# jgrss/cultionet

Measured on AMD Instinct MI355X. Metric: train_chips_per_sec, higher is better.
Workload: dtype f32

## Files before the change

### cultionet_amd/csrc/cn_conv.hip

```cpp
#include "cn_common.h"
#include "cn_conv_geom.h"
#include "cn_profile.h"

#include <cstdlib>

#define KC 8

static int cn_reduce_slices(const CnConvGeom& g, hipStream_t stream);

template <int TN, int TM>
__device__ __forceinline__ void cn_igemm_epilogue(const CnConvGeom& g, const f32x16 (&acc)[TN][TM],
                                                  const bool (&pix_ok)[TM], const int (&out_off)[TM], int co_base,
                                                  int half, int grp, int split, int b,
                                                  const float* __restrict__ bias, float* __restrict__ y) {
  const int HWout = g.Hout * g.Wout;
  const bool sliced = g.slice_stride != 0;
  float* yb = sliced ? g.part + (long)(grp * g.splits + split) * g.slice_stride + (long)b * g.Cout * HWout
                     : y + (long)b * g.ybs;
  const bool first = split == 0;
#pragma unroll
  for (int tn = 0; tn < TN; ++tn) {
#pragma unroll
    for (int r = 0; r < 16; ++r) {
      const int co = co_base + tn * 32 + (r & 3) + 8 * (r >> 2) + 4 * half;
// ... 166 lines not shown
  {                                                                                                        \
    const float* wrow = w_lds + ((t_) * KC + half) * NT + wn * (TN * 32) + l31;                            \
    _Pragma("unroll") for (int tn = 0; tn < TN; ++tn) opa[bf_][tn] = wrow[(2 * (cp_)) * NT + tn * 32];     \
    opb[bf_][0] = in_lds[pix_lds[0] + (2 * (cp_)) * plane + (toff_)];                                      \
    opb[bf_][1] = in_lds[pix_lds[1] + (2 * (cp_)) * plane + (toff_)];                                      \
  }
#define CN_MFMA(bf_)                                                                                       \
  _Pragma("unroll") for (int tn = 0; tn < TN; ++tn) _Pragma("unroll") for (int tm = 0; tm < 2; ++tm)       \
      acc[tn][tm] = __builtin_amdgcn_mfma_f32_32x32x2f32(opa[bf_][tn], opb[bf_][tm], acc[tn][tm], 0, 0, 0);
      int toff_cur = tap_lds[0];
      CN_LOAD_OPS(0, 0, 0, toff_cur);
#pragma unroll 1
      for (int t = 0; t < ntaps; ++t) {
        const int toff_nxt = (t + 1 < ntaps) ? tap_lds[t + 1] : 0;
        CN_LOAD_OPS(1, t, 1, toff_cur);
        CN_MFMA(0);
        CN_LOAD_OPS(0, t, 2, toff_cur);
        CN_MFMA(1);
        CN_LOAD_OPS(1, t, 3, toff_cur);
        CN_MFMA(0);
        if (t + 1 < ntaps) CN_LOAD_OPS(0, t + 1, 0, toff_nxt);
        CN_MFMA(1);
        toff_cur = toff_nxt;
      }
#undef CN_LOAD_OPS
#undef CN_MFMA
    }
#undef CN_PREFETCH
  }

  cn_igemm_epilogue<TN, 2>(g, acc, pix_ok, out_off, n0 + wn * (TN * 32), half, grp, split, b, bias, y);
}

template <int WAVES_N, int TN, int TM, int NV, int RP>
__global__ __launch_bounds__(256, (NV <= 1 ? 2 : 1)) void cn_conv_igemm_vec_kernel(const CnConvGeom g) {
  constexpr int WAVES_M = 4 / WAVES_N;
  constexpr int MT = WAVES_M * TM * 32;
  constexpr int NT = WAVES_N * TN * 32;
  constexpr int WI = (CN_MAX_TAPS * KC * (NT / 4) + 255) / 256;
  constexpr int VS = NV * 1024;
  constexpr bool PADR = RP == 1 || RP == 2;
  constexpr int ODD = RP == 3 ? 1 : 0;
  constexpr int VSS = VS + ODD;
  extern __shared__ __attribute__((aligned(16))) float smem[];
  float* in_lds = smem;
  float* w_lds = smem + g.w_lds_off;
  int* tap_lds = reinterpret_cast<int*>(smem + g.tap_lds_off);

  const int tid = threadIdx.x, lane = tid & 63, wid = tid >> 6;
  const int half = lane >> 5, l31 = lane & 31;
  const int wm = wid / WAVES_N, wn = wid % WAVES_N;

  int bx, by, split;
  if (!cn_xcd_block(g.grid_x, g.grid_y, g.grid_x * g.grid_y * g.splits, bx, by, split)) return;
  int ci_ = 0;
  if (g.interleave) {
    ci_ = bx % g.ncls;
  } else {
#pragma unroll 1
    for (int c = 1; c < g.ncls; ++c)
      if (bx >= g.cls[c].block_begin) ci_ = c;
  }
  const int grp = g.cls[ci_].grp;
  const float* __restrict__ x = g.gx[grp];
  const float* __restrict__ wp = g.gwp[grp];
  const float* __restrict__ bias = g.gbias[grp];
  float* __restrict__ y = g.gy[grp];
  const int Hg = g.cls[ci_].Hg, Wg = g.cls[ci_].Wg, ntaps = g.cls[ci_].ntaps;
  const int vplane = g.cls[ci_].vplane;
  const int min_dy = g.cls[ci_].min_dy, min_dx = g.cls[ci_].min_dx;
  const int oy0 = g.cls[ci_].oy0, ox0 = g.cls[ci_].ox0;
  const int tiles_per_img = g.cls[ci_].tiles_per_img;
  const int tile = g.interleave ? bx / g.ncls : bx - g.cls[ci_].block_begin;
  const int b = tile / tiles_per_img;
  const int m0 = (tile - b * tiles_per_img) * MT;
  const int Win = g.Win;
  const int pitch = PADR ? ((Win + 3) / 4 * 4 + 4) : Win;
  if (tid < ntaps) {
    tap_lds[tid] = PADR ? (g.cls[ci_].dy[tid] - min_dy) * pitch + g.cls[ci_].dx[tid]
                      : (g.cls[ci_].dy[tid] - min_dy) * Win + (g.cls[ci_].dx[tid] - min_dx);
    tap_lds[CN_MAX_TAPS + tid] = g.cls[ci_].wt[tid];
    tap_lds[2 * CN_MAX_TAPS + tid] = g.cls[ci_].dx[tid];
  }
  __syncthreads();
  const int n0 = by * NT;
  const int Mimg = Hg * Wg;
  const int gy0 = m0 / Wg;
  const int HWin = g.Hin * Win;
  const int start = PADR ? (gy0 * g.is + min_dy) * Win : (gy0 * g.is + min_dy) * Win + min_dx;
  const int f0 = (start >> 2) << 2;
  const int sh = start - f0;

  int goff[NV];
  int ldst[NV];
  int ldst2[NV];
#pragma unroll
  for (int i = 0; i < NV; ++i) {
    const int e4 = 4 * (tid + i * 256) - (PADR ? sh : 0);
    const int lim = PADR ? g.cls[ci_].rows * Win : vplane;
    ldst[i] = 0;
    ldst2[i] = 0;
    if (e4 + 3 >= 0 && e4 < lim) {
      const int fq = start + e4 - (PADR ? 0 : sh);
      goff[i] = (fq >= 0 && (ODD ? fq < HWin : fq + 3 < HWin)) ? fq : -1;
      if (RP == 1) {
        const int r = e4 / Win;
        ldst[i] = r * pitch + 4 + (e4 - r * Win);
      } else if (RP == 2) {
        const int ea = e4 < 0 ? e4 + 2 : e4, eb = e4 + 2;
        const int ra = ea / Win, rb = eb / Win;
        ldst[i] = e4 < 0 ? -1 : ra * pitch + 4 + (ea - ra * Win);
        ldst2[i] = eb < lim ? rb * pitch + 4 + (eb - rb * Win) : -1;
      } else {
        ldst[i] = e4;
      }
    } else {
      goff[i] = -2;
    }
  }
  if (PADR) {
    for (int e = tid; e < KC * VS; e += 256) in_lds[e] = 0.f;
  }

  int pix_lds[TM], out_off[TM];
  unsigned colmask[TM];
  bool pix_ok[TM];
#pragma unroll
  for (int tm = 0; tm < TM; ++tm) {
    const int p = m0 + wm * (TM * 32) + tm * 32 + l31;
    pix_ok[tm] = p < Mimg;
    const int pc = pix_ok[tm] ? p : Mimg - 1;
    const int gy = pc / Wg, gx = pc - gy * Wg;
    pix_lds[tm] = PADR ? ((gy - gy0) * g.is) * pitch + 4 + gx * g.is + half * VS
                     : ((gy - gy0) * g.is) * Win + gx * g.is + sh + half * VSS;
    out_off[tm] = (gy * g.os + oy0) * g.Wout + gx * g.os + ox0;
    unsigned m = 0;
    for (int t = 0; t < ntaps; ++t) {
      const int ix = gx * g.is + tap_lds[2 * CN_MAX_TAPS + t];
      if (ix >= 0 && ix < Win) m |= 1u << t;
    }
    colmask[tm] = m;
  }

  f32x16 acc[TN][TM];
#pragma unroll
  for (int tn = 0; tn < TN; ++tn)
#pragma unroll
    for (int tm = 0; tm < TM; ++tm)
#pragma unroll
      for (int r = 0; r < 16; ++r) acc[tn][tm][r] = 0.f;
  const float* xb = x + (long)b * g.xbs;
  const int nw4 = ntaps * KC * (NT / 4);
  const int nchunks = (g.Cin + KC - 1) / KC;
  int ch = split * g.chunks_per_split;
  int ch_end = ch + g.chunks_per_split;
  if (ch_end > nchunks) ch_end = nchunks;

  if (ntaps > 0 && ch < ch_end) {
    f32x4 xin[KC][NV];
    f32x4 win[WI];
    constexpr unsigned CN_OOB = 0x80000000u;
    const __amdgpu_buffer_rsrc_t xrs =
        __builtin_amdgcn_make_buffer_rsrc(const_cast<float*>(xb), 0, 0x7fffffff, 0x00020000);
    const __amdgpu_buffer_rsrc_t wrs =
        __builtin_amdgcn_make_buffer_rsrc(const_cast<float*>(wp), 0, 0x7fffffff, 0x00020000);
    unsigned xo[NV], wo[WI];
#pragma unroll
    for (int i = 0; i < NV; ++i) xo[i] = goff[i] >= 0 ? (unsigned)goff[i] * 4u : CN_OOB;
#pragma unroll
    for (int j = 0; j < WI; ++j) {
      const int f = tid + j * 256;
      wo[j] = CN_OOB;
      if (f < nw4) {
        const int row = f / (NT / 4), c4 = f - row * (NT / 4);
        const int t = row / KC, ci = row - t * KC;
        wo[j] = (unsigned)(((tap_lds[CN_MAX_TAPS + t] * g.Kpad + ci) * g.Npad + n0 + c4 * 4) * 4);
      }
    }
#define CN_PREFETCH_V(c0_)                                                                                 \
  {                                                                                                        \
    const int c0 = (c0_);                                                                                  \
    _Pragma("unroll") for (int ci = 0; ci < KC; ++ci) {                                                    \
      if ((c0 + ci) < g.Cin) {                                                           \
        const int so = ODD ? (((c0 + ci) * HWin) & ~3) * 4 : (c0 + ci) * HWin * 4;                                                               \
        _Pragma("unroll") for (int i = 0; i < NV; ++i)                                                     \
            xin[ci][i] = __builtin_bit_cast(f32x4, __builtin_amdgcn_raw_buffer_load_b128(xrs, xo[i], so, 0)); \
      } else {                                                                                             \
        _Pragma("unroll") for (int i = 0; i < NV; ++i) xin[ci][i] = f32x4{0.f, 0.f, 0.f, 0.f};             \
      }                                                                                                    \
    }                                                                                                      \
    const int wso = c0 * g.Npad * 4;                                                                       \
    _Pragma("unroll") for (int j = 0; j < WI; ++j)                                                         \
        win[j] = __builtin_bit_cast(f32x4, __builtin_amdgcn_raw_buffer_load_b128(wrs, wo[j], wso, 0));     \
  }
    CN_PREFETCH_V(ch * KC);
    for (; ch < ch_end; ++ch) {
      __syncthreads();
#pragma unroll
      for (int ci = 0; ci < KC; ++ci)
#pragma unroll
        for (int i = 0; i < NV; ++i)
          if (goff[i] != -2) {
            if (RP == 2) {
              if (ldst[i] >= 0) *reinterpret_cast<float2*>(in_lds + ci * VS + ldst[i]) = make_float2(xin[ci][i][0], xin[ci][i][1]);
              if (ldst2[i] >= 0) *reinterpret_cast<float2*>(in_lds + ci * VS + ldst2[i]) = make_float2(xin[ci][i][2], xin[ci][i][3]);
            } else if (ODD) {
              f32x4 v = xin[ci][i];
              const int dl = ci & 3;
              const bool first = dl > 0 && goff[i] == 0;
              const bool last = dl < 3 && goff[i] == HWin - 1;
#pragma unroll
              for (int j = 0; j < 4; ++j)
                if ((first && j < dl) || (last && j > dl)) v[j] = 0.f;
              *reinterpret_cast<f32x4*>(in_lds + ci * VS + (ci & ~3) + ldst[i]) = v;
            } else {
              *reinterpret_cast<f32x4*>(in_lds + ci * VS + ldst[i]) = xin[ci][i];
            }
          }
#pragma unroll
      for (int j = 0; j < WI; ++j) {
        const int f = tid + j * 256;
        if (f < nw4) *reinterpret_cast<f32x4*>(w_lds + f * 4) = win[j];
      }
      __syncthreads();
      if (ch + 1 < ch_end) CN_PREFETCH_V((ch + 1) * KC);
#pragma unroll 1
      for (int t = 0; t < ntaps; ++t) {
        const int toff = tap_lds[t];
        const float* wrow = w_lds + (t * KC + half) * NT + wn * (TN * 32) + l31;
        const float* brow[TM];
        int msk[TM];
#pragma unroll
        for (int tm = 0; tm < TM; ++tm) {
          brow[tm] = in_lds + pix_lds[tm] + toff;
          msk[tm] = PADR ? -1 : __builtin_amdgcn_sbfe((int)colmask[tm], t, 1);
        }
#pragma unroll
        for (int cp = 0; cp < KC / 2; ++cp) {
          float a[TN], bb[TM];
#pragma unroll
          for (int tn = 0; tn < TN; ++tn) a[tn] = wrow[(2 * cp) * NT + tn * 32];
#pragma unroll
          for (int tm = 0; tm < TM; ++tm)
            bb[tm] = PADR ? brow[tm][(2 * cp) * VS] : __int_as_float(__float_as_int(brow[tm][(2 * cp) * VSS]) & msk[tm]);
#pragma unroll
          for (int tn = 0; tn < TN; ++tn)
#pragma unroll
            for (int tm = 0; tm < TM; ++tm)
              acc[tn][tm] = __builtin_amdgcn_mfma_f32_32x32x2f32(a[tn], bb[tm], acc[tn][tm], 0, 0, 0);
        }
      }
    }
#undef CN_PREFETCH_V
  }

  cn_igemm_epilogue<TN, TM>(g, acc, pix_ok, out_off, n0 + wn * (TN * 32), half, grp, split, b, bias, y);
}

__global__ void cn_pack_weights_kernel(const float* __restrict__ w, float* __restrict__ wp, int T, int K,
                                       int N, int Kpad, int Npad, long sk, long sn, long st) {
  const long total = (long)T * Kpad * Npad;
  for (long i = blockIdx.x * (long)blockDim.x + threadIdx.x; i < total; i += (long)gridDim.x * blockDim.x) {
    const int n = (int)(i % Npad);
    const long r = i / Npad;
    const int k = (int)(r % Kpad);
    const int t = (int)(r / Kpad);
    wp[i] = (k < K && n < N) ? w[k * sk + n * sn + t * st] : 0.f;
  }
}

struct CnPackDesc {
  const float* w;
  float* wp;
  int T, K, N, Kpad, Npad;
  long sk, sn, st;
};

#define CN_PK_TS 32
#define CN_PK_PITCH (32 * CN_MAX_TAPS + 1)
__global__ __launch_bounds__(256) void cn_pack_weights_batched_kernel(const CnPackDesc* __restrict__ descs) {
  __shared__ float tile[CN_PK_TS * CN_PK_PITCH];
  const CnPackDesc d = descs[blockIdx.y];
  const bool n_slow = d.sn > d.sk;
  const long ss = n_slow ? d.sn : d.sk, sm = n_slow ? d.sk : d.sn;
  const int S = n_slow ? d.N : d.K, M = n_slow ? d.K : d.N;
  const int Spad = n_slow ? d.Npad : d.Kpad, Mpad = n_slow ? d.Kpad : d.Npad;
  if (d.T > CN_MAX_TAPS || d.st != 1 || sm != d.T) {
    const long total = (long)d.T * d.Kpad * d.Npad;
    for (long i = blockIdx.x * (long)blockDim.x + threadIdx.x; i < total; i += (long)gridDim.x * blockDim.x) {
// ... 139 lines not shown
      if (t == 0 || k.dy[t] > max_dy) max_dy = k.dy[t];
      if (t == 0 || k.dx[t] > max_dx) max_dx = k.dx[t];
    }
    const int rows = (rows_g - 1) * g.is + (max_dy - k.min_dy) + 1;
    k.pitch = (k.Wg - 1) * g.is + (max_dx - k.min_dx) + 1;
    k.plane = rows * k.pitch;
    k.vplane = (rows * g.Win + (max_dx - k.min_dx) + 4 + 3) / 4 * 4;
    k.rows = rows;
    {
      const int rpitch = (g.Win + 3) / 4 * 4 + 4;
      if ((rows + 1) * rpitch + 4 > p.max_rplane) p.max_rplane = (rows + 1) * rpitch + 4;
    }
    if (-k.min_dx > p.max_absdx) p.max_absdx = -k.min_dx;
    if (max_dx > p.max_absdx) p.max_absdx = max_dx;
    k.tiles_per_img = (Mimg + MT - 1) / MT;
    k.block_begin = p.total_tiles;
    p.total_tiles += g.B * k.tiles_per_img;
    if (k.plane > p.max_plane) p.max_plane = k.plane;
    if (k.vplane > p.max_vplane) p.max_vplane = k.vplane;
    if (k.ntaps > p.max_taps) p.max_taps = k.ntaps;
    p.flops += 2.0 * g.B * Mimg * (double)g.Cout * g.Cin * k.ntaps;
  }
  g.interleave = 0;
  if (g.ncls > 1 && g.want_interleave) {
    bool same = true;
    for (int c = 1; c < g.ncls; ++c) same = same && g.cls[c].tiles_per_img == g.cls[0].tiles_per_img;
    g.interleave = same ? 1 : 0;
  }
  return p;
}

struct CnChoice { int cfg, splits, cps; double cost; };

static double cn_launch_cost(long blocks, int cps, double mt_units, int splits, double out_elems) {
  const double F = 273.0, R = 170.0;
  const double c1 = 36.7 + 0.614 * mt_units, c2 = 30.0 + 1.19 * mt_units;
  const long full = blocks / 512, rem = blocks % 512;
  double c = full * (F + cps * c2);
  if (rem > 0) c += F + cps * (rem > 256 ? c2 : c1);
  if (splits > 1) c += R + out_elems * 4.0 * (2.0 * splits + 1.0) / 8.0e6 * (128.0 / 7.5);
  return c;
}

static thread_local float* g_conv_ws;
static thread_local long g_conv_ws_floats;

static CnChoice cn_choose(const CnConvGeom& g0, const int* mts, int ncfg, int NT, bool allow_split) {
  const int nchunks = (g0.Cin + KC - 1) / KC;
  const int ny = (g0.Cout + NT - 1) / NT;
  const int G = g0.G > 0 ? g0.G : 1;
  const double out_elems = (double)g0.B * g0.Cout * g0.Hout * g0.Wout * (g0.shared_y ? 1 : G);
  CnChoice best = {0, 1, nchunks > 0 ? nchunks : 1, 1e300};
  int forced = 0;
  {
    static const char* dbg = getenv("CN_DBG_SPLITS");
    if (dbg) forced = atoi(dbg) < 1 ? 1 : atoi(dbg);
  }
  long ws_cap = 32;
  if (g_conv_ws != nullptr) {
    const long stride = ((long)g0.B * g0.Cout * g0.Hout * g0.Wout + 3) / 4 * 4;
    ws_cap = g_conv_ws_floats / (stride * G);
  }
  int forced_cfg = -1;
  {
    static const char* dbgc = getenv("CN_DBG_CFG");
    if (dbgc) forced_cfg = atoi(dbgc);
  }
  for (int i = 0; i < ncfg; ++i) {
    if (forced_cfg >= 0 && i != (forced_cfg < ncfg ? forced_cfg : ncfg - 1)) continue;
    CnConvGeom gi = g0;
    const CnPlan p = cn_plan(gi, mts[i]);
    if (p.total_tiles <= 0) continue;
    const long base = (long)p.total_tiles * ny;
    int max_splits = (allow_split && p.max_taps > 0 && nchunks >= 4) ? nchunks / 2 : 1;
    if (max_splits > 32) max_splits = 32;
    if (max_splits > ws_cap) max_splits = ws_cap < 1 ? 1 : (int)ws_cap;
    const double taps = p.total_tiles > 0 ? p.flops / (2.0 * g0.Cout * g0.Cin * (double)mts[i] * p.total_tiles) : 9.0;
    const double chunk_units = (double)mts[i] * NT / 128.0 * (taps < 9.0 ? taps : 9.0) / 9.0;
    for (int sp = 1; sp <= max_splits; ++sp) {
      if (forced && sp != (forced > max_splits ? max_splits : forced)) continue;
      const int cps = (nchunks + sp - 1) / sp;
      const int splits = (nchunks + cps - 1) / cps;
      if (splits != sp && !forced) continue;
      const double cost = cn_launch_cost(base * splits, cps, chunk_units, splits, out_elems);
      if (cost < best.cost * (i == best.cfg ? 1.0 : 0.98)) best = {i, splits, cps, cost};
    }
  }
  return best;
}


#include <mutex>
#include <unordered_map>
namespace {
struct CnWs { float* p; long n; };
std::mutex g_ws_mu;
std::unordered_map<void*, CnWs> g_ws_by_stream;
}

extern "C" int cn_conv_set_workspace(void* stream, float* ws, long ws_floats) {
// ... 119 lines not shown
    CN_GO(4, 1);
  }
  if (rp == 2) {
    if (img <= 1024) CN_GO(1, 2);
    if (img <= 2048) CN_GO(2, 2);
    CN_GO(4, 2);
  }
  if (rp == 3) {
    if (img <= 1024) CN_GO(1, 3);
    if (img <= 2048) CN_GO(2, 3);
    CN_GO(4, 3);
  }
  if (img <= 1024) CN_GO(1, 0);
  if (img <= 2048) CN_GO(2, 0);
  CN_GO(4, 0);
#undef CN_GO
}

template <int WAVES_N, int TN>
static int cn_launch_dword_cfg(const float* x, const float* wp, const float* bias, float* y, CnConvGeom& g,
                               int splits, int cps, hipStream_t stream) {
  constexpr int MT = (4 / WAVES_N) * 64;
  const CnPlan p = cn_plan(g, MT);
  if (p.total_tiles <= 0) return CN_OK;
  if (p.max_plane > 12 * 256) return CN_ERR_LDS;
  g.w_lds_off = (KC * p.max_plane + 3) / 4 * 4;
  const int rc = cn_finish_split(g, p, splits, cps, y, stream);
  if (rc != CN_OK) return rc;
  if (p.max_plane <= 3 * 256)
    return cn_launch_igemm_t<WAVES_N, TN, 3>(x, wp, bias, y, g, p.total_tiles, p.max_taps, splits, p.flops, stream);
  if (p.max_plane <= 6 * 256)
    return cn_launch_igemm_t<WAVES_N, TN, 6>(x, wp, bias, y, g, p.total_tiles, p.max_taps, splits, p.flops, stream);
  return cn_launch_igemm_t<WAVES_N, TN, 12>(x, wp, bias, y, g, p.total_tiles, p.max_taps, splits, p.flops, stream);
}

struct CnGemm1x1 {
  int B, Cin, Cout, HW, Kpad, Npad, tiles_per_img, grid_x, grid_y, accumulate;
  long xbs, ybs;
};
#define KC1 32

template <int TM>
__global__ __launch_bounds__(256) void cn_conv1x1_kernel(const float* __restrict__ x, const float* __restrict__ wp,
                                                        const float* __restrict__ bias, float* __restrict__ y,
                                                        const CnGemm1x1 g) {
  constexpr int MT = TM * 32, NT = 128;
  constexpr int NA = KC1 * NT / 4 / 256;
  constexpr int NB = (KC1 * MT / 4 + 255) / 256;
  __shared__ __attribute__((aligned(16))) float a_lds[KC1 * NT];
  __shared__ __attribute__((aligned(16))) float b_lds[KC1 * MT];
  int bx, by, bz;
  if (!cn_xcd_block(g.grid_x, g.grid_y, g.grid_x * g.grid_y, bx, by, bz)) return;
  const int tid = threadIdx.x, lane = tid & 63, wn = tid >> 6;
  const int half = lane >> 5, l31 = lane & 31;
  const int b = bx / g.tiles_per_img;
  const int p0 = (bx - b * g.tiles_per_img) * MT;
  const int n0 = by * NT;
  const float* xb = x + (long)b * g.xbs;

  f32x16 acc[TM];
#pragma unroll
  for (int tm = 0; tm < TM; ++tm)
#pragma unroll
    for (int r = 0; r < 16; ++r) acc[tm][r] = 0.f;

  f32x4 ra[NA], rb[NB];
// ... 146 lines not shown
             hipEventElapsedTime(&ms, e0, e1) == hipSuccess;
      }
      if (ok && ms < best_ms) { best_ms = ms; best = c; }
    }
  }
  (void)hipEventDestroy(e0);
  (void)hipEventDestroy(e1);
  return best;
}

int cn_conv_igemm_launch(CnConvGeom& g, hipStream_t stream) {
  if (g.ncls < 1 || g.ncls > CN_MAX_CLASSES || g.B <= 0 || g.G < 1) return g.B <= 0 ? CN_OK : CN_ERR_ARG;
  g.splits = 1;
  const float* x = g.gx[0]; const float* wp = g.gwp[0]; const float* bias = g.gbias[0]; float* y = g.gy[0];
  g.Kpad = cn_conv_kpad(g.Cin);
  g.Npad = cn_conv_npad(g.Cout);
  const int nt = cn_pick_nt(g.Cout);
  const bool dense_out = g.ybs == (long)g.Cout * g.Hout * g.Wout;
  const bool ws_fits = g_conv_ws != nullptr &&
                       (((long)g.B * g.Cout * g.Hout * g.Wout + 3) / 4 * 4) * g.G * 32 <= g_conv_ws_floats;
  const bool allow_split = dense_out || g.accumulate || ws_fits;
  if (g.G > 1 && g.shared_y && !allow_split) return CN_ERR_ARG;
  const int hw4 = (int)(((long)g.Hin * g.Win) % 4);
  g.odd_planes = (hw4 == 1 && !(g.is > 1 && (long)g.Hin * g.Win > 4096)) ? 1 : 0;
  bool vec = (hw4 == 0 || g.odd_planes) && (g.xbs % 4 == 0);
  if (g.is > 1 && (long)g.Hin * g.Win > 4096) vec = false;
  if ((long)g.Cin * g.Hin * g.Win * 4 >= (1L << 31) || (long)CN_MAX_TAPS * cn_conv_kpad(g.Cin) * g.Npad * 4 >= (1L << 31))
    return CN_ERR_ARG;
  for (int i = 0; i < g.G; ++i) vec = vec && ((reinterpret_cast<uintptr_t>(g.gx[i]) & 15) == 0);
  if (vec) {
    CnConvGeom t = g;
    vec = cn_plan(t, 256).max_vplane <= 4 * 1024;
  }
  static const int mts128[3] = {128, 96, 160};
  static const int mts128d[1] = {128};
  static const int mts256[1] = {256};
  const int* mts = nt == 128 ? (vec ? mts128 : mts128d) : mts256;
  const int ncfg = (nt == 128 && vec) ? 3 : 1;
  auto run = [&](const CnChoice& c, CnConvGeom& gg) -> int {
    if (nt == 128) {
      if (vec) {
        switch (c.cfg) {
          case 1: return cn_launch_vec_cfg<4, 1, 3>(x, wp, bias, y, gg, c.splits, c.cps, stream);
          case 2: return cn_launch_vec_cfg<4, 1, 5>(x, wp, bias, y, gg, c.splits, c.cps, stream);
          default: return cn_launch_vec_cfg<2, 2, 2>(x, wp, bias, y, gg, c.splits, c.cps, stream);
        }
      }
      return cn_launch_dword_cfg<2, 2>(x, wp, bias, y, gg, c.splits, c.cps, stream);
    }
    int rc;
    if (nt == 64) {
      if (vec) return cn_launch_vec_cfg<1, 2, 2>(x, wp, bias, y, gg, c.splits, c.cps, stream);
      rc = cn_launch_dword_cfg<1, 2>(x, wp, bias, y, gg, c.splits, c.cps, stream);
    } else {
      if (vec) return cn_launch_vec_cfg<1, 1, 2>(x, wp, bias, y, gg, c.splits, c.cps, stream);
      rc = cn_launch_dword_cfg<1, 1>(x, wp, bias, y, gg, c.splits, c.cps, stream);
    }
    if (rc == CN_ERR_LDS) {
      CnConvGeom g2 = gg;
      rc = cn_launch_dword_cfg<2, 2>(x, wp, bias, y, g2, c.splits, c.cps, stream);
    }
    return rc;
  };
  CnChoice c = cn_choose(g, mts, ncfg, nt, allow_split);
  if (g_autotune) {
    std::lock_guard<std::mutex> lk(g_tune_mu);
// ... 81 lines not shown
  if (stride < 1 || G * stride * stride > CN_MAX_CLASSES) return CN_ERR_ARG;
  for (int i = 0; i < G; ++i)
    if (khs[i] * kws[i] > CN_MAX_TAPS || khs[i] < 1 || kws[i] < 1) return CN_ERR_ARG;
  if (G == 1 && khs[0] == 1 && kws[0] == 1 && stride == 1 && pads[0] == 0 && Ho == Hs && Wo == Ws) {
    const int r1 = cn_conv1x1_launch(srcs[0], sbs, wps[0], biases ? biases[0] : nullptr, outs[0], obs, B, Csrc,
                                     Hs * Ws, Cdst, accumulate, stream);
    if (r1 != CN_ERR_ARG) return r1;
  }
  CnConvGeom g = {};
  const int rc = cn_set_groups(g, G, srcs, wps, biases, outs);
  if (rc != CN_OK) return rc;
  g.B = B; g.Cin = Csrc; g.Hin = Hs; g.Win = Ws; g.Cout = Cdst; g.Hout = Ho; g.Wout = Wo;
  g.xbs = sbs; g.ybs = obs; g.is = 1; g.os = stride;
  g.accumulate = accumulate;
  int nc = 0;
  for (int gi = 0; gi < G; ++gi) {
    const int pad = pads[gi], dil = dils[gi], KH = khs[gi], KW = kws[gi];
    if (dil < 1) return CN_ERR_ARG;
    for (int py = 0; py < stride; ++py)
      for (int px = 0; px < stride; ++px) {
        CnConvClass& k = g.cls[nc];
        k.grp = gi;
        k.Hg = cn_parity_extent(Ho, py, stride);
        k.Wg = cn_parity_extent(Wo, px, stride);
        if (k.Hg <= 0 || k.Wg <= 0) continue;
        k.oy0 = py; k.ox0 = px;
        k.ntaps = cn_parity_taps(py, px, KH, KW, stride, pad, dil, k.dy, k.dx, k.wt);
        ++nc;
      }
  }
  g.ncls = nc;
  if (nc == 0) return CN_OK;
  cn_sort_heavy_first(g.cls, nc);
  g.want_interleave = stride > 1 ? 1 : 0;
  return cn_conv_igemm_launch(g, stream);
}

static int cn_scatter_conv(const float* src, long sbs, const float* wp, const float* bias, float* out, long obs,
                           int B, int Csrc, int Hs, int Ws, int Cdst, int Ho, int Wo, int KH, int KW,
                           int stride, int pad, int dil, int accumulate, hipStream_t stream) {
  return cn_scatter_conv_g(1, &src, sbs, &wp, &bias, &out, obs, B, Csrc, Hs, Ws, Cdst, Ho, Wo, &KH, &KW, stride, &pad,
                           &dil, accumulate, stream);
}

extern "C" int cn_conv2d_bwd_data_f32(const float* dy, long dybs, const float* wp_t, float* dx, long dxbs,
                                      int B, int Cin, int Hin, int Win, int Cout, int KH, int KW, int stride,
                                      int pad, int dil, int accumulate, void* stream) {
  cn_bind_ws(stream);
  if (stride < 1) return CN_ERR_ARG;
  const int Hout = cn_conv_out(Hin, KH, stride, pad, dil);
  const int Wout = cn_conv_out(Win, KW, stride, pad, dil);
  return cn_scatter_conv(dy, dybs, wp_t, nullptr, dx, dxbs, B, Cout, Hout, Wout, Cin, Hin, Win, KH, KW, stride,
                         pad, dil, accumulate, (hipStream_t)stream);
}

extern "C" int cn_conv2d_fwd_grouped_f32(int G, const float* const* xs, long xbs, const float* const* wps,
                                         const float* const* biases, float* const* ys, long ybs, int B, int Cin,
                                         int Hin, int Win, int Cout, int KH, int KW, int stride, const int* pads,
                                         const int* dils, int accumulate, void* stream) {
  cn_bind_ws(stream);
  if (G < 1 || G > CN_MAX_GROUPS) return CN_ERR_ARG;
  if (stride < 1) return CN_ERR_ARG;
  const int Hout = cn_conv_out(Hin, KH, stride, pads[0], dils[0]);
  const int Wout = cn_conv_out(Win, KW, stride, pads[0], dils[0]);
  for (int i = 1; i < G; ++i)
    if (cn_conv_out(Hin, KH, stride, pads[i], dils[i]) != Hout ||
// ... 98 lines not shown
```

### cultionet_amd/csrc/cn_conv_geom.h

```cpp
#pragma once
#define CN_MAX_TAPS 9
#define CN_MAX_CLASSES 16
#define CN_MAX_GROUPS 4

struct CnConvClass {
  int Hg, Wg;
  int oy0, ox0;
  int ntaps;
  int dy[CN_MAX_TAPS], dx[CN_MAX_TAPS], wt[CN_MAX_TAPS];
  int min_dy, min_dx;
  int pitch, plane;
  int vplane;
  int rows;
  int tiles_per_img;
  int block_begin;
  int grp;
};

struct CnConvGeom {
  int B, Cin, Hin, Win;
  int Cout, Hout, Wout;
  long xbs, ybs;
  int is, os;
  int Kpad, Npad;
  int w_lds_off;
  int tap_lds_off;
  int chunks_per_split;
  int atomic_out;
  int accumulate, has_bias;
  int G, splits, shared_y;
  int odd_planes;
  int want_interleave;
  int interleave;
  float* part;
  long slice_stride;
  int grid_x, grid_y;
  const float* gx[CN_MAX_GROUPS];
  const float* gwp[CN_MAX_GROUPS];
  const float* gbias[CN_MAX_GROUPS];
  float* gy[CN_MAX_GROUPS];
  int ncls;
  CnConvClass cls[CN_MAX_CLASSES];
};

static inline int cn_conv_out(int in, int k, int stride, int pad, int dil) {
  return (in + 2 * pad - dil * (k - 1) - 1) / stride + 1;
}
static inline int cn_convt_out(int in, int k, int stride, int pad, int out_pad) {
  return (in - 1) * stride - 2 * pad + k + out_pad;
}
static inline int cn_floordiv(int a, int b) { return (a >= 0) ? a / b : -((-a + b - 1) / b); }

static inline int cn_gather_taps(int KH, int KW, int pad, int dil, int* dy, int* dx, int* wt) {
  for (int ky = 0; ky < KH; ++ky)
    for (int kx = 0; kx < KW; ++kx) {
      const int t = ky * KW + kx;
      dy[t] = ky * dil - pad; dx[t] = kx * dil - pad; wt[t] = t;
    }
  return KH * KW;
}

static inline int cn_parity_extent(int out, int p, int stride) { return (out - p + stride - 1) / stride; }

// ... 26 lines not shown
```

Before: 384.7.

## Add cell-based kernel for stride-2 3x3 transposed conv scatter

Adds a specialized kernel for stride-2, 3x3, pad-1 scatter convolutions (transposed conv / backward data). Each block computes all four output parity classes from one shared 2x2 input neighbourhood, so the input tile and weights are staged once instead of once per parity class. The staging code is factored into reusable helpers, and a separate cost-model fit picks the tile size and split count for the new path. The new path adds code complexity and relies on the cost model and the edge masking being correct.

```diff
diff --git a/cultionet_amd/csrc/cn_conv.hip b/cultionet_amd/csrc/cn_conv.hip
--- a/cultionet_amd/csrc/cn_conv.hip
+++ b/cultionet_amd/csrc/cn_conv.hip
@@ -222,6 +222,115 @@
   cn_igemm_epilogue<TN, 2>(g, acc, pix_ok, out_off, n0 + wn * (TN * 32), half, grp, split, b, bias, y);
 }
 
+constexpr unsigned CN_OOB = 0x80000000u;
+
+template <int NV, int RP>
+__device__ __forceinline__ void cn_stage_decode(int tid, int start, int sh, int lim, int Win, int pitch, int HWin,
+                                                int (&goff)[NV], int (&ldst)[NV], int (&ldst2)[NV],
+                                                unsigned (&xo)[NV]) {
+  constexpr bool PADR = RP == 1 || RP == 2;
+  constexpr int ODD = RP == 3 ? 1 : 0;
+#pragma unroll
+  for (int i = 0; i < NV; ++i) {
+    const int e4 = 4 * (tid + i * 256) - (PADR ? sh : 0);
+    ldst[i] = 0;
+    ldst2[i] = 0;
+    if (e4 + 3 >= 0 && e4 < lim) {
+      const int fq = start + e4 - (PADR ? 0 : sh);
+      goff[i] = (fq >= 0 && (ODD ? fq < HWin : fq + 3 < HWin)) ? fq : -1;
+      if (RP == 1) {
+        const int r = e4 / Win;
+        ldst[i] = r * pitch + 4 + (e4 - r * Win);
+      } else if (RP == 2) {
+        const int ea = e4 < 0 ? e4 + 2 : e4, eb = e4 + 2;
+        const int ra = ea / Win, rb = eb / Win;
+        ldst[i] = e4 < 0 ? -1 : ra * pitch + 4 + (ea - ra * Win);
+        ldst2[i] = eb < lim ? rb * pitch + 4 + (eb - rb * Win) : -1;
+      } else {
+        ldst[i] = e4;
+      }
+    } else {
+      goff[i] = -2;
+    }
+    xo[i] = goff[i] >= 0 ? (unsigned)goff[i] * 4u : CN_OOB;
+  }
+}
+
+template <int NV, int RP>
+__device__ __forceinline__ void cn_stage_prefetch(f32x4 (&xin)[KC][NV], __amdgpu_buffer_rsrc_t xrs,
+                                                  const unsigned (&xo)[NV], int c0, int Cin, int HWin) {
+  constexpr int ODD = RP == 3 ? 1 : 0;
+#pragma unroll
+  for (int ci = 0; ci < KC; ++ci) {
+    const bool in = (c0 + ci) < Cin;
+    const int so = !in ? 0 : ODD ? (((c0 + ci) * HWin) & ~3) * 4 : (c0 + ci) * HWin * 4;
+#pragma unroll
+    for (int i = 0; i < NV; ++i)
+      xin[ci][i] = __builtin_bit_cast(f32x4, __builtin_amdgcn_raw_buffer_load_b128(xrs, in ? xo[i] : CN_OOB, so, 0));
+  }
+}
+
+template <int NV, int RP>
+__device__ __forceinline__ void cn_stage_store(float* in_lds, const f32x4 (&xin)[KC][NV], const int (&goff)[NV],
+                                               const int (&ldst)[NV], const int (&ldst2)[NV], int HWin) {
+  constexpr int ODD = RP == 3 ? 1 : 0;
+  constexpr int VS = NV * 1024;
+#pragma unroll
+  for (int ci = 0; ci < KC; ++ci)
+#pragma unroll
+    for (int i = 0; i < NV; ++i)
+      if (goff[i] != -2) {
+        if (RP == 2) {
+          if (ldst[i] >= 0) *reinterpret_cast<float2*>(in_lds + ci * VS + ldst[i]) = make_float2(xin[ci][i][0], xin[ci][i][1]);
+          if (ldst2[i] >= 0) *reinterpret_cast<float2*>(in_lds + ci * VS + ldst2[i]) = make_float2(xin[ci][i][2], xin[ci][i][3]);
+        } else if (ODD) {
+          f32x4 v = xin[ci][i];
+          const int dl = ci & 3;
+          const bool first = dl > 0 && goff[i] == 0;
+          const bool last = dl < 3 && goff[i] == HWin - 1;
+#pragma unroll
+          for (int j = 0; j < 4; ++j)
+            if ((first && j < dl) || (last && j > dl)) v[j] = 0.f;
+          *reinterpret_cast<f32x4*>(in_lds + ci * VS + (ci & ~3) + ldst[i]) = v;
+        } else {
+          *reinterpret_cast<f32x4*>(in_lds + ci * VS + ldst[i]) = xin[ci][i];
+        }
+      }
+}
+
+template <int WI, int NT>
+__device__ __forceinline__ void cn_wstage_decode(unsigned (&wo)[WI], int tid, int nw4, const int* tap_lds, int Kpad,
+                                                 int Npad, int n0) {
+#pragma unroll
+  for (int j = 0; j < WI; ++j) {
+    const int f = tid + j * 256;
+    wo[j] = CN_OOB;
+    if (f < nw4) {
+      const int row = f / (NT / 4), c4 = f - row * (NT / 4);
+      const int t = row / KC, ci = row - t * KC;
+      wo[j] = (unsigned)(((tap_lds[CN_MAX_TAPS + t] * Kpad + ci) * Npad + n0 + c4 * 4) * 4);
+    }
+  }
+}
+
+template <int WI>
+__device__ __forceinline__ void cn_wstage_prefetch(f32x4 (&win)[WI], __amdgpu_buffer_rsrc_t wrs,
+                                                   const unsigned (&wo)[WI], int c0, int Npad) {
+  const int wso = c0 * Npad * 4;
+#pragma unroll
+  for (int j = 0; j < WI; ++j)
+    win[j] = __builtin_bit_cast(f32x4, __builtin_amdgcn_raw_buffer_load_b128(wrs, wo[j], wso, 0));
+}
+
+template <int WI>
+__device__ __forceinline__ void cn_wstage_store(float* w_lds, const f32x4 (&win)[WI], int tid, int nw4) {
+#pragma unroll
+  for (int j = 0; j < WI; ++j) {
+    const int f = tid + j * 256;
+    if (f < nw4) *reinterpret_cast<f32x4*>(w_lds + f * 4) = win[j];
+  }
+}
+
 template <int WAVES_N, int TN, int TM, int NV, int RP>
 __global__ __launch_bounds__(256, (NV <= 1 ? 2 : 1)) void cn_conv_igemm_vec_kernel(const CnConvGeom g) {
   constexpr int WAVES_M = 4 / WAVES_N;
@@ -284,30 +393,8 @@
   int goff[NV];
   int ldst[NV];
   int ldst2[NV];
-#pragma unroll
-  for (int i = 0; i < NV; ++i) {
-    const int e4 = 4 * (tid + i * 256) - (PADR ? sh : 0);
-    const int lim = PADR ? g.cls[ci_].rows * Win : vplane;
-    ldst[i] = 0;
-    ldst2[i] = 0;
-    if (e4 + 3 >= 0 && e4 < lim) {
-      const int fq = start + e4 - (PADR ? 0 : sh);
-      goff[i] = (fq >= 0 && (ODD ? fq < HWin : fq + 3 < HWin)) ? fq : -1;
-      if (RP == 1) {
-        const int r = e4 / Win;
-        ldst[i] = r * pitch + 4 + (e4 - r * Win);
-      } else if (RP == 2) {
-        const int ea = e4 < 0 ? e4 + 2 : e4, eb = e4 + 2;
-        const int ra = ea / Win, rb = eb / Win;
-        ldst[i] = e4 < 0 ? -1 : ra * pitch + 4 + (ea - ra * Win);
-        ldst2[i] = eb < lim ? rb * pitch + 4 + (eb - rb * Win) : -1;
-      } else {
-        ldst[i] = e4;
-      }
-    } else {
-      goff[i] = -2;
-    }
-  }
+  unsigned xo[NV];
+  cn_stage_decode<NV, RP>(tid, start, sh, PADR ? g.cls[ci_].rows * Win : vplane, Win, pitch, HWin, goff, ldst, ldst2, xo);
   if (PADR) {
     for (int e = tid; e < KC * VS; e += 256) in_lds[e] = 0.f;
   }
@@ -349,71 +436,23 @@
   if (ntaps > 0 && ch < ch_end) {
     f32x4 xin[KC][NV];
     f32x4 win[WI];
-    constexpr unsigned CN_OOB = 0x80000000u;
     const __amdgpu_buffer_rsrc_t xrs =
         __builtin_amdgcn_make_buffer_rsrc(const_cast<float*>(xb), 0, 0x7fffffff, 0x00020000);
     const __amdgpu_buffer_rsrc_t wrs =
         __builtin_amdgcn_make_buffer_rsrc(const_cast<float*>(wp), 0, 0x7fffffff, 0x00020000);
-    unsigned xo[NV], wo[WI];
-#pragma unroll
-    for (int i = 0; i < NV; ++i) xo[i] = goff[i] >= 0 ? (unsigned)goff[i] * 4u : CN_OOB;
-#pragma unroll
-    for (int j = 0; j < WI; ++j) {
-      const int f = tid + j * 256;
-      wo[j] = CN_OOB;
-      if (f < nw4) {
-        const int row = f / (NT / 4), c4 = f - row * (NT / 4);
-        const int t = row / KC, ci = row - t * KC;
-        wo[j] = (unsigned)(((tap_lds[CN_MAX_TAPS + t] * g.Kpad + ci) * g.Npad + n0 + c4 * 4) * 4);
-      }
-    }
-#define CN_PREFETCH_V(c0_)                                                                                 \
-  {                                                                                                        \
-    const int c0 = (c0_);                                                                                  \
-    _Pragma("unroll") for (int ci = 0; ci < KC; ++ci) {                                                    \
-      if ((c0 + ci) < g.Cin) {                                                           \
-        const int so = ODD ? (((c0 + ci) * HWin) & ~3) * 4 : (c0 + ci) * HWin * 4;                                                               \
-        _Pragma("unroll") for (int i = 0; i < NV; ++i)                                                     \
-            xin[ci][i] = __builtin_bit_cast(f32x4, __builtin_amdgcn_raw_buffer_load_b128(xrs, xo[i], so, 0)); \
-      } else {                                                                                             \
-        _Pragma("unroll") for (int i = 0; i < NV; ++i) xin[ci][i] = f32x4{0.f, 0.f, 0.f, 0.f};             \
-      }                                                                                                    \
-    }                                                                                                      \
-    const int wso = c0 * g.Npad * 4;                                                                       \
-    _Pragma("unroll") for (int j = 0; j < WI; ++j)                                                         \
-        win[j] = __builtin_bit_cast(f32x4, __builtin_amdgcn_raw_buffer_load_b128(wrs, wo[j], wso, 0));     \
-  }
-    CN_PREFETCH_V(ch * KC);
+    unsigned wo[WI];
+    cn_wstage_decode<WI, NT>(wo, tid, nw4, tap_lds, g.Kpad, g.Npad, n0);
+    cn_stage_prefetch<NV, RP>(xin, xrs, xo, ch * KC, g.Cin, HWin);
+    cn_wstage_prefetch<WI>(win, wrs, wo, ch * KC, g.Npad);
     for (; ch < ch_end; ++ch) {
       __syncthreads();
-#pragma unroll
-      for (int ci = 0; ci < KC; ++ci)
-#pragma unroll
-        for (int i = 0; i < NV; ++i)
-          if (goff[i] != -2) {
-            if (RP == 2) {
-              if (ldst[i] >= 0) *reinterpret_cast<float2*>(in_lds + ci * VS + ldst[i]) = make_float2(xin[ci][i][0], xin[ci][i][1]);
-              if (ldst2[i] >= 0) *reinterpret_cast<float2*>(in_lds + ci * VS + ldst2[i]) = make_float2(xin[ci][i][2], xin[ci][i][3]);
-            } else if (ODD) {
-              f32x4 v = xin[ci][i];
-              const int dl = ci & 3;
-              const bool first = dl > 0 && goff[i] == 0;
-              const bool last = dl < 3 && goff[i] == HWin - 1;
-#pragma unroll
-              for (int j = 0; j < 4; ++j)
-                if ((first && j < dl) || (last && j > dl)) v[j] = 0.f;
-              *reinterpret_cast<f32x4*>(in_lds + ci * VS + (ci & ~3) + ldst[i]) = v;
-            } else {
-              *reinterpret_cast<f32x4*>(in_lds + ci * VS + ldst[i]) = xin[ci][i];
-            }
-          }
-#pragma unroll
-      for (int j = 0; j < WI; ++j) {
-        const int f = tid + j * 256;
-        if (f < nw4) *reinterpret_cast<f32x4*>(w_lds + f * 4) = win[j];
+      cn_stage_store<NV, RP>(in_lds, xin, goff, ldst, ldst2, HWin);
+      cn_wstage_store<WI>(w_lds, win, tid, nw4);
+      __syncthreads();
+      if (ch + 1 < ch_end) {
+        cn_stage_prefetch<NV, RP>(xin, xrs, xo, (ch + 1) * KC, g.Cin, HWin);
+        cn_wstage_prefetch<WI>(win, wrs, wo, (ch + 1) * KC, g.Npad);
       }
-      __syncthreads();
-      if (ch + 1 < ch_end) CN_PREFETCH_V((ch + 1) * KC);
 #pragma unroll 1
       for (int t = 0; t < ntaps; ++t) {
         const int toff = tap_lds[t];
@@ -441,10 +480,147 @@
         }
       }
     }
-#undef CN_PREFETCH_V
   }
 
   cn_igemm_epilogue<TN, TM>(g, acc, pix_ok, out_off, n0 + wn * (TN * 32), half, grp, split, b, bias, y);
+}
+
+template <int TMC, int RP>
+__global__ __launch_bounds__(256, 2) void cn_conv_cells_kernel(const CnConvGeom g) {
+  constexpr int MT = TMC * 32;
+  constexpr int NT = 128;
+  constexpr int WI = (CN_MAX_TAPS * KC * (NT / 4) + 255) / 256;
+  constexpr int VS = 1024;
+  constexpr bool PADR = RP == 1 || RP == 2;
+  constexpr int VSS = VS + (RP == 3 ? 1 : 0);
+  extern __shared__ __attribute__((aligned(16))) float smem[];
+  float* in_lds = smem;
+  float* w_lds = smem + g.w_lds_off;
+  int* tap_lds = reinterpret_cast<int*>(smem + g.tap_lds_off);
+
+  const int tid = threadIdx.x, lane = tid & 63, wid = tid >> 6;
+  const int half = lane >> 5, l31 = lane & 31;
+  const int wn = wid;
+
+  int bx, by, split;
+  if (!cn_xcd_block(g.grid_x, g.grid_y, g.grid_x * g.grid_y * g.splits, bx, by, split)) return;
+  const float* __restrict__ x = g.gx[0];
+  const float* __restrict__ wp = g.gwp[0];
+  const float* __restrict__ bias = g.gbias[0];
+  float* __restrict__ y = g.gy[0];
+  const int tiles_per_img = g.cls[0].tiles_per_img;
+  const int b = __builtin_amdgcn_readfirstlane(bx / tiles_per_img);
+  const int m0 = (bx - b * tiles_per_img) * MT;
+  const int Win = g.Win;
+  const int pitch = PADR ? ((Win + 3) / 4 * 4 + 4) : Win;
+  if (tid < CN_MAX_TAPS) tap_lds[CN_MAX_TAPS + tid] = tid;
+  __syncthreads();
+  const int n0 = by * NT;
+  const int HWin = g.Hin * Win;
+  const int gy0 = m0 / Win;
+  const int start = gy0 * Win;
+  const int f0 = (start >> 2) << 2;
+  const int sh = start - f0;
+
+  int goff[1], ldst[1], ldst2[1];
+  unsigned xo[1];
+  cn_stage_decode<1, RP>(tid, start, sh, PADR ? g.cls[0].rows * Win : g.cls[0].vplane, Win, pitch, HWin, goff, ldst,
+                         ldst2, xo);
+  if (PADR) {
+    for (int e = tid; e < KC * VS; e += 256) in_lds[e] = 0.f;
+  }
+
+  int pix_lds[TMC], mskx[TMC];
+#pragma unroll
+  for (int tm = 0; tm < TMC; ++tm) {
+    const int p = m0 + tm * 32 + l31;
+    const int pc = p < HWin ? p : HWin - 1;
+    const int cy = pc / Win, cx = pc - cy * Win;
+    pix_lds[tm] = PADR ? (cy - gy0) * pitch + 4 + cx + half * VS : (cy - gy0) * Win + cx + sh + half * VSS;
+    mskx[tm] = (PADR || cx + 1 < Win) ? -1 : 0;
+  }
+
+  f32x16 acc[4][1][TMC];
+#pragma unroll
+  for (int c = 0; c < 4; ++c)
+#pragma unroll
+    for (int tm = 0; tm < TMC; ++tm)
+#pragma unroll
+      for (int r = 0; r < 16; ++r) acc[c][0][tm][r] = 0.f;
+  const float* xb = x + (long)b * g.xbs;
+  const int nw4 = CN_MAX_TAPS * KC * (NT / 4);
+  const int nchunks = (g.Cin + KC - 1) / KC;
+  int ch = split * g.chunks_per_split;
+  int ch_end = ch + g.chunks_per_split;
+  if (ch_end > nchunks) ch_end = nchunks;
+
+  if (ch < ch_end) {
+    f32x4 xin[KC][1];
+    f32x4 win[WI];
+    const __amdgpu_buffer_rsrc_t xrs =
+        __builtin_amdgcn_make_buffer_rsrc(const_cast<float*>(xb), 0, 0x7fffffff, 0x00020000);
+    const __amdgpu_buffer_rsrc_t wrs =
+        __builtin_amdgcn_make_buffer_rsrc(const_cast<float*>(wp), 0, 0x7fffffff, 0x00020000);
+    unsigned wo[WI];
+    cn_wstage_decode<WI, NT>(wo, tid, nw4, tap_lds, g.Kpad, g.Npad, n0);
+    cn_stage_prefetch<1, RP>(xin, xrs, xo, ch * KC, g.Cin, HWin);
+    cn_wstage_prefetch<WI>(win, wrs, wo, ch * KC, g.Npad);
+    const float* wrow = w_lds + half * NT + wn * 32 + l31;
+    const float* brow0[TMC];
+#pragma unroll
+    for (int tm = 0; tm < TMC; ++tm) brow0[tm] = in_lds + pix_lds[tm];
+    for (; ch < ch_end; ++ch) {
+      __syncthreads();
+      cn_stage_store<1, RP>(in_lds, xin, goff, ldst, ldst2, HWin);
+      cn_wstage_store<WI>(w_lds, win, tid, nw4);
+      __syncthreads();
+      if (ch + 1 < ch_end) {
+        cn_stage_prefetch<1, RP>(xin, xrs, xo, (ch + 1) * KC, g.Cin, HWin);
+        cn_wstage_prefetch<WI>(win, wrs, wo, (ch + 1) * KC, g.Npad);
+      }
+#pragma unroll
+      for (int cp = 0; cp < KC / 2; ++cp) {
+        float a[CN_MAX_TAPS], bb[TMC][4];
+#pragma unroll
+        for (int t = 0; t < CN_MAX_TAPS; ++t) a[t] = wrow[(t * KC + 2 * cp) * NT];
+#pragma unroll
+        for (int tm = 0; tm < TMC; ++tm) {
+          const float* r0 = brow0[tm] + (2 * cp) * VSS;
+          const float* r1 = r0 + pitch;
+          bb[tm][0] = r0[0];
+          bb[tm][1] = __int_as_float(__float_as_int(r0[1]) & mskx[tm]);
+          bb[tm][2] = r1[0];
+          bb[tm][3] = __int_as_float(__float_as_int(r1[1]) & mskx[tm]);
+        }
+#pragma unroll
+        for (int ky = 0; ky < 3; ++ky)
+#pragma unroll
+          for (int kx = 0; kx < 3; ++kx) {
+            const int c = (ky != 1 ? 2 : 0) + (kx != 1 ? 1 : 0), s = (ky == 0 ? 2 : 0) + (kx == 0 ? 1 : 0);
+#pragma unroll
+            for (int tm = 0; tm < TMC; ++tm)
+              acc[c][0][tm] = __builtin_amdgcn_mfma_f32_32x32x2f32(a[ky * 3 + kx], bb[tm][s], acc[c][0][tm], 0, 0, 0);
+          }
+      }
+    }
+  }
+
+#pragma unroll
+  for (int c = 0; c < 4; ++c) {
+    const int py = c >> 1, px = c & 1;
+    bool ok[TMC];
+    int out_off[TMC];
+#pragma unroll
+    for (int tm = 0; tm < TMC; ++tm) {
+      const int p = m0 + tm * 32 + l31;
+      const int pc = p < HWin ? p : HWin - 1;
+      const int cy = pc / Win, cx = pc - cy * Win;
+      const int oy = 2 * cy + py, ox = 2 * cx + px;
+      ok[tm] = p < HWin && oy < g.Hout && ox < g.Wout;
+      out_off[tm] = oy * g.Wout + ox;
+    }
+    cn_igemm_epilogue<1, TMC>(g, acc[c], ok, out_off, n0 + wn * 32, half, 0, split, b, bias, y);
+  }
 }
 
 __global__ void cn_pack_weights_kernel(const float* __restrict__ w, float* __restrict__ wp, int T, int K,
@@ -650,18 +826,38 @@
 
 struct CnChoice { int cfg, splits, cps; double cost; };
 
-static double cn_launch_cost(long blocks, int cps, double mt_units, int splits, double out_elems) {
-  const double F = 273.0, R = 170.0;
-  const double c1 = 36.7 + 0.614 * mt_units, c2 = 30.0 + 1.19 * mt_units;
+struct CnCostFit { double F, a1, b1, a2, b2; };
+static const CnCostFit CN_FIT_CLASS = {273.0, 36.7, 0.614, 30.0, 1.19};
+static const CnCostFit CN_FIT_CELLS = {130.0, 22.5, 0.614, 16.7, 1.19};
+
+static double cn_launch_cost(long blocks, int cps, double mt_units, int splits, double out_elems,
+                             const CnCostFit& f = CN_FIT_CLASS) {
+  const double R = 170.0;
+  const double c1 = f.a1 + f.b1 * mt_units, c2 = f.a2 + f.b2 * mt_units;
   const long full = blocks / 512, rem = blocks % 512;
-  double c = full * (F + cps * c2);
-  if (rem > 0) c += F + cps * (rem > 256 ? c2 : c1);
+  double c = full * (f.F + cps * c2);
+  if (rem > 0) c += f.F + cps * (rem > 256 ? c2 : c1);
   if (splits > 1) c += R + out_elems * 4.0 * (2.0 * splits + 1.0) / 8.0e6 * (128.0 / 7.5);
   return c;
 }
 
 static thread_local float* g_conv_ws;
 static thread_local long g_conv_ws_floats;
+
+static int cn_dbg_splits() {
+  static const char* dbg = getenv("CN_DBG_SPLITS");
+  return dbg ? (atoi(dbg) < 1 ? 1 : atoi(dbg)) : 0;
+}
+static int cn_dbg_cfg() {
+  static const char* dbgc = getenv("CN_DBG_CFG");
+  return dbgc ? atoi(dbgc) : -1;
+}
+
+static long cn_ws_cap(const CnConvGeom& g0) {
+  if (g_conv_ws == nullptr) return 32;
+  const long stride = ((long)g0.B * g0.Cout * g0.Hout * g0.Wout + 3) / 4 * 4;
+  return g_conv_ws_floats / (stride * (g0.G > 0 ? g0.G : 1));
+}
 
 static CnChoice cn_choose(const CnConvGeom& g0, const int* mts, int ncfg, int NT, bool allow_split) {
   const int nchunks = (g0.Cin + KC - 1) / KC;
@@ -669,21 +865,9 @@
   const int G = g0.G > 0 ? g0.G : 1;
   const double out_elems = (double)g0.B * g0.Cout * g0.Hout * g0.Wout * (g0.shared_y ? 1 : G);
   CnChoice best = {0, 1, nchunks > 0 ? nchunks : 1, 1e300};
-  int forced = 0;
-  {
-    static const char* dbg = getenv("CN_DBG_SPLITS");
-    if (dbg) forced = atoi(dbg) < 1 ? 1 : atoi(dbg);
-  }
-  long ws_cap = 32;
-  if (g_conv_ws != nullptr) {
-    const long stride = ((long)g0.B * g0.Cout * g0.Hout * g0.Wout + 3) / 4 * 4;
-    ws_cap = g_conv_ws_floats / (stride * G);
-  }
-  int forced_cfg = -1;
-  {
-    static const char* dbgc = getenv("CN_DBG_CFG");
-    if (dbgc) forced_cfg = atoi(dbgc);
-  }
+  const int forced = cn_dbg_splits();
+  const long ws_cap = cn_ws_cap(g0);
+  const int forced_cfg = cn_dbg_cfg();
   for (int i = 0; i < ncfg; ++i) {
     if (forced_cfg >= 0 && i != (forced_cfg < ncfg ? forced_cfg : ncfg - 1)) continue;
     CnConvGeom gi = g0;
@@ -869,6 +1053,96 @@
   if (p.max_plane <= 6 * 256)
     return cn_launch_igemm_t<WAVES_N, TN, 6>(x, wp, bias, y, g, p.total_tiles, p.max_taps, splits, p.flops, stream);
   return cn_launch_igemm_t<WAVES_N, TN, 12>(x, wp, bias, y, g, p.total_tiles, p.max_taps, splits, p.flops, stream);
+}
+
+template <int TMC, int RP>
+static int cn_launch_cells_t(CnConvGeom& g, int total_tiles, int splits, double flops, hipStream_t stream) {
+  constexpr int NT = 128;
+  g.tap_lds_off = g.w_lds_off + CN_MAX_TAPS * KC * NT;
+  const size_t lds = (size_t)(g.tap_lds_off + 3 * CN_MAX_TAPS + 1) * sizeof(float);
+  if (lds > 80 * 1024) return CN_ERR_LDS;
+  static bool attr_set = false;
+  if (!attr_set) {
+    (void)hipFuncSetAttribute((const void*)cn_conv_cells_kernel<TMC, RP>,
+                              hipFuncAttributeMaxDynamicSharedMemorySize, 80 * 1024);
+    attr_set = true;
+  }
+  g.grid_x = total_tiles;
+  g.grid_y = (g.Cout + NT - 1) / NT;
+  g.splits = splits < 1 ? 1 : splits;
+  dim3 grid(cn_xcd_grid((long)g.grid_x * g.grid_y * g.splits));
+  cn_prof_name("cn_conv_cells_kernel<%d, %d>", TMC, RP);
+  cn_prof_desc("cells<%d,%d> B%d %d->%d %dx%d->%dx%d taps9 cls4 grid%dx%dx%d", TMC, RP, g.B, g.Cin, g.Cout,
+               g.Hin, g.Win, g.Hout, g.Wout, total_tiles, g.grid_y, splits);
+  cn_prof_bytes(4.0 * ((double)g.B * g.Cin * g.Hin * g.Win + (double)g.B * g.Cout * g.Hout * g.Wout +
+                       (double)CN_MAX_TAPS * g.Cin * g.Cout));
+  cn_prof_before(stream);
+  CN_LAUNCH((cn_conv_cells_kernel<TMC, RP>), grid, dim3(256), lds, stream, g);
+  cn_prof_after(stream, 0, flops);
+  const int rrc = cn_reduce_slices(g, stream);
+  return rrc != CN_OK ? rrc : cn_check_launch();
+}
+
+static int cn_try_cells(const CnConvGeom& g, bool allow_split, hipStream_t stream, bool& taken) {
+  taken = false;
+  if (cn_pick_nt(g.Cout) != 128) return CN_OK;
+  const int rp = g.odd_planes ? 3 : (g.Win % 4 == 0 ? 1 : (g.Win % 2 == 0 ? 2 : 0));
+  if (rp == 0) return CN_OK;
+  const int nchunks = (g.Cin + KC - 1) / KC;
+  const double out_elems = (double)g.B * g.Cout * g.Hout * g.Wout;
+  double flops;
+  {
+    CnConvGeom t = g;
+    flops = cn_plan(t, 128).flops;
+  }
+  CnConvGeom gc = g;
+  gc.ncls = 1;
+  gc.want_interleave = 0;
+  gc.is = 1;
+  {
+    CnConvClass& k = gc.cls[0];
+    k = CnConvClass{};
+    k.Hg = g.Hin; k.Wg = g.Win; k.ntaps = 4;
+    for (int s = 0; s < 4; ++s) { k.dy[s] = s >> 1; k.dx[s] = s & 1; k.wt[s] = s; }
+  }
+  const long ws_cap = cn_ws_cap(g);
+  const int forced = cn_dbg_splits(), forced_cfg = cn_dbg_cfg();
+  CnChoice best = {-1, 1, nchunks > 0 ? nchunks : 1, 1e300};
+  CnConvGeom gbest = gc;
+  CnPlan pbest = {};
+  for (int i = 0; i < 2; ++i) {
+    if (forced_cfg >= 0 && i != (forced_cfg < 2 ? forced_cfg : 1)) continue;
+    const int MT = i == 0 ? 64 : 32;
+    CnConvGeom gi = gc;
+    CnPlan p = cn_plan(gi, MT);
+    if (p.total_tiles <= 0) continue;
+    gi.cls[0].vplane += 4;
+    if ((rp == 3 ? gi.cls[0].vplane : p.max_rplane) > 1024) continue;
+    const long base = (long)p.total_tiles * ((g.Cout + 127) / 128);
+    int max_splits = (allow_split && nchunks >= 4) ? nchunks / 2 : 1;
+    if (max_splits > 32) max_splits = 32;
+    if (max_splits > ws_cap) max_splits = ws_cap < 1 ? 1 : (int)ws_cap;
+    for (int sp = 1; sp <= max_splits; ++sp) {
+      if (forced && sp != (forced > max_splits ? max_splits : forced)) continue;
+      const int cps = (nchunks + sp - 1) / sp;
+      const int splits = (nchunks + cps - 1) / cps;
+      if (splits != sp && !forced) continue;
+      const double cost = cn_launch_cost(base * splits, cps, (double)MT, splits, out_elems, CN_FIT_CELLS);
+      if (cost < best.cost) { best = {i, splits, cps, cost}; gbest = gi; pbest = p; }
+    }
+  }
+  if (best.cfg < 0) return CN_OK;
+  taken = true;
+  gbest.w_lds_off = KC * 1024 + (rp == 3 ? 16 : 0);
+  const int rc = cn_finish_split(gbest, pbest, best.splits, best.cps, gbest.gy[0], stream);
+  if (rc != CN_OK) return rc;
+#define CN_CELLS_GO(TMC_)                                                                                    \
+  return rp == 1   ? cn_launch_cells_t<TMC_, 1>(gbest, pbest.total_tiles, best.splits, flops, stream)        \
+         : rp == 2 ? cn_launch_cells_t<TMC_, 2>(gbest, pbest.total_tiles, best.splits, flops, stream)        \
+                   : cn_launch_cells_t<TMC_, 3>(gbest, pbest.total_tiles, best.splits, flops, stream)
+  if (best.cfg == 0) CN_CELLS_GO(2);
+  CN_CELLS_GO(1);
+#undef CN_CELLS_GO
 }
 
 struct CnGemm1x1 {
@@ -1081,6 +1355,11 @@
     CnConvGeom t = g;
     vec = cn_plan(t, 256).max_vplane <= 4 * 1024;
   }
+  if (g.cells && vec) {
+    bool taken = false;
+    const int rc = cn_try_cells(g, allow_split, stream, taken);
+    if (taken) return rc;
+  }
   static const int mts128[3] = {128, 96, 160};
   static const int mts128d[1] = {128};
   static const int mts256[1] = {256};
@@ -1228,6 +1507,8 @@
   g.ncls = nc;
   if (nc == 0) return CN_OK;
   cn_sort_heavy_first(g.cls, nc);
+  g.cells = (G == 1 && stride == 2 && khs[0] == 3 && kws[0] == 3 && pads[0] == 1 && dils[0] == 1 &&
+             Hs == (Ho + 1) / 2 && Ws == (Wo + 1) / 2) ? 1 : 0;
   g.want_interleave = stride > 1 ? 1 : 0;
   return cn_conv_igemm_launch(g, stream);
 }
diff --git a/cultionet_amd/csrc/cn_conv_geom.h b/cultionet_amd/csrc/cn_conv_geom.h
--- a/cultionet_amd/csrc/cn_conv_geom.h
+++ b/cultionet_amd/csrc/cn_conv_geom.h
@@ -29,6 +29,7 @@
   int atomic_out;
   int accumulate, has_bias;
   int G, splits, shared_y;
+  int cells;
   int odd_planes;
   int want_interleave;
   int interleave;
```

After: 384.1 (median of 2 runs). About the same (-0.2%).
